# gisbi-kim/navtech-radar-slam

Hardware: AMD Instinct MI355X
Metric: sc_loop_queries_per_sec_vs_10k_scan_db (higher is better)
Workload: dtype f16 filter + f64 exact

## Files before the change

include/rsx_diag.h:

```cpp
#ifndef RSX_DIAG_H
#define RSX_DIAG_H

#include "rsx.h"

#ifdef __cplusplus
extern "C" {
#endif

int rsx_selftest_firewall(int kind);

int rsx_frontend_read_images(rsx_frontend *h, int32_t image, float *out_cart, float *out_blur);

int rsx_cen2018_gauss_weights(int32_t sigma_gauss, float *out, int32_t max);
int rsx_cen2018_debug_image(rsx_cen2018 *h, const uint8_t *img, int32_t row_stride, int32_t col_offset, const rsx_cen2018_params *params,
                            float *out_mean, float *out_sigma, float *out_p, float *out_y);

int rsx_sc_ringkey_tree_layout(const float *keys20, int64_t n, int32_t *out_vind, int32_t *out_n_nodes, int32_t *out_depth);

int rsx_sc_filter_bounds(rsx_sc *h, const float *q_descs, int32_t nq, float *out_lb);
double rsx_sc_filter_eps(void);

#define RSX_SC_WINDOW_P 320
#define RSX_SC_WINDOW_MARGIN 1.25e-3f
int rsx_sc_window_previews(rsx_sc *h, const float *q_descs, int32_t nq, int32_t k, int32_t *out_slots, float *out_pv,
                           int32_t *out_kstar, int32_t *out_shift_mask, int32_t *out_counts);

const char *rsx_sc_dominant_kernel_name(void);
const char *rsx_sc_profiled_kernel_name(rsx_sc *h);
int rsx_sc_profile_enable(rsx_sc *h, int on);
int rsx_sc_profile_read(rsx_sc *h, int64_t *launches, double *total_ms);
typedef struct {
  uint32_t struct_size;
  uint32_t reserved;
  int64_t candidates;
  int64_t exact_evals;
  int64_t queries_rescored;
  int64_t window_previews;
  int64_t valu_previews;
  int64_t exact_window_shifts;
} rsx_sc_rescoring_stats;
int rsx_sc_profile_read_rescoring(rsx_sc *h, rsx_sc_rescoring_stats *out);

#ifdef __cplusplus
}
#endif
#endif
```

navtech-radar-slam_amd/_rsx.py:

```python
import ctypes as C
import os

import numpy as np

_HERE = os.path.dirname(os.path.abspath(__file__))
LIB_PATH = os.environ.get("RSX_LIB_PATH") or os.path.join(_HERE, "librsx.so")

NUM_RING, NUM_SECTOR, DESC_SIZE, MAX_TOPK = 20, 60, 1200, 32
MODE_CANDIDATE, MODE_EXHAUSTIVE = 0, 1
FILTER_AUTO, FILTER_OFF, FILTER_FORCE, FILTER_Q1 = 0, 1, 2, 3
KIND_AUTO, KIND_DIRECT, KIND_SPECTRAL, KIND_SPECTRAL2 = 0, 1, 2, 3
SUM_EIGEN_SSE2, SUM_SEQ, SUM_EIGEN_AVX_FMA, SUM_EIGEN34_AVX_FMA = 0, 1, 2, 3
default_filter_kind = KIND_AUTO

HIT_DTYPE = np.dtype([("dist", "<f8"), ("index", "<i4"), ("shift", "<i4")])


class RsxError(RuntimeError):
    def __init__(self, status, msg):
        super().__init__(f"rsx status {status}: {msg}")
        self.status = status


class ScParams(C.Structure):
    _fields_ = [
        ("lidar_height", C.c_double),
        ("max_radius", C.c_double),
        ("num_exclude_recent", C.c_int32),
        ("num_candidates", C.c_int32),
        ("search_ratio", C.c_double),
        ("dist_thres", C.c_double),
        ("tree_making_period", C.c_int32),
        ("device", C.c_int32),
        ("shard_rank", C.c_int32),
        ("shard_world", C.c_int32),
        ("capacity_hint", C.c_int64),
        ("filter_mode", C.c_int32),
        ("filter_kind", C.c_int32),
        ("sum_order", C.c_int32),
    ]


class RescoringStats(C.Structure):
    _fields_ = [("struct_size", C.c_uint32), ("reserved", C.c_uint32), ("candidates", C.c_int64), ("exact_evals", C.c_int64),
                ("queries_rescored", C.c_int64), ("window_previews", C.c_int64), ("valu_previews", C.c_int64),
                ("exact_window_shifts", C.c_int64)]


ORORA_PMC = 4
ORORA_PMC_EXACT = 8
ORORA_PMC_PROVEN, ORORA_PMC_PASSTHROUGH, ORORA_PMC_NO_WORKSPACE, ORORA_PMC_MAXIMUM, ORORA_PMC_BUDGET = 1, 2, 4, 8, 16
PMC_INFO_DTYPE = np.dtype([("size", "<i4"), ("max_core", "<i4"), ("seeds", "<i4"), ("flags", "<i4")])


class ScDetection(C.Structure):
    _fields_ = [("loop_id", C.c_int32), ("yaw_diff_rad", C.c_float), ("min_dist", C.c_double), ("nn_idx", C.c_int32),
                ("query_idx", C.c_int32), ("searched", C.c_int32), ("reserved", C.c_int32), ("dist_thres", C.c_double)]


class OroraParams(C.Structure):
    _fields_ = [("tim_noise_bound", C.c_double), ("noise_bound_radial", C.c_double),
                ("noise_bound_tangential", C.c_double), ("gnc_factor", C.c_double),
                ("cost_threshold", C.c_double), ("max_iterations", C.c_int32), ("flags", C.c_int32)]


class IcpParams(C.Structure):
    _fields_ = [("max_corr_dist", C.c_double), ("transformation_epsilon", C.c_double),
                ("euclidean_fitness_epsilon", C.c_double), ("max_iterations", C.c_int32), ("flags", C.c_int32)]


class IcpResult(C.Structure):
    _fields_ = [("transform", C.c_float * 16), ("fitness", C.c_double), ("iterations", C.c_int32),
                ("converged", C.c_int32), ("state", C.c_int32), ("reserved", C.c_int32)]


class LoopVerifyParams(C.Structure):
    _fields_ = [("history_keyframe_search_num", C.c_int32), ("leaf", C.c_float), ("fitness_threshold", C.c_double), ("icp", IcpParams)]


class LoopVerifyResult(C.Structure):
    _fields_ = [("accepted", C.c_int32), ("converged", C.c_int32), ("iterations", C.c_int32), ("state", C.c_int32),
                ("fitness", C.c_double), ("transform", C.c_float * 16),
                ("x", C.c_float), ("y", C.c_float), ("z", C.c_float), ("roll", C.c_float), ("pitch", C.c_float), ("yaw", C.c_float),
                ("relative", C.c_double * 16), ("n_source", C.c_int64), ("n_target", C.c_int64)]


class FrontendParams(C.Structure):
    _fields_ = [("cart_pixel_width", C.c_int32), ("cart_resolution", C.c_float), ("ratio", C.c_float), ("flags", C.c_int32)]


class Cen2019Params(C.Structure):
    _fields_ = [("max_points", C.c_int32), ("min_range", C.c_int32)]


class Cen2018Params(C.Structure):
    _fields_ = [("zq", C.c_float), ("sigma_gauss", C.c_int32), ("min_range", C.c_int32), ("reserved", C.c_int32)]


class OroraResult(C.Structure):
# ... 261 lines not shown
```

navtech-radar-slam_amd/csrc/sc_api.cpp:

```cpp
#include <cmath>
#include <cstdio>
#include <cstdlib>
#include <cstring>
#include <mutex>
#include <new>
#include <string>
#include <vector>

#include "rsx_common.h"
#include "sc_kernels.h"
#include "sc_plan.h"
#include "sc_kdtree.h"
#include "loopverify.h"
#include "voxelgrid.h"

namespace rsx {
std::string &last_error() {
  static thread_local std::string e;
  return e;
}
}

using namespace rsx;
using namespace rsx::sc;
// ... 1489 lines not shown
    int count = 0;
    for (int p = 0; p < nparts; p++)
      for (int i = 0; i < k; i++) {
        const rsx_sc_hit &r = parts[((size_t)p * nq + q) * k + i];
        if (!(r.dist < 10000000)) continue;
        int pos = count < k ? count : k;
        while (pos > 0 && ((r.dist < o[pos - 1].dist) || (r.dist == o[pos - 1].dist && r.index < o[pos - 1].index))) pos--;
        if (pos >= k) continue;
        int last = count < k ? count : k - 1;
        for (int j = last; j > pos; j--) o[j] = o[j - 1];
        o[pos] = r;
        if (count < k) count++;
      }
    for (int i = count; i < k; i++) {
      o[i].dist = 10000000;
      o[i].index = 0;
      o[i].shift = 0;
    }
  }
  return RSX_OK;
} RSX_CATCH_ALL

int rsx_sc_merge_topk_device(rsx_sc *h, const rsx_sc_hit *d_parts, int32_t nparts, int32_t nq, int32_t k,
                             rsx_sc_hit *d_out, void *stream) try {
  if (!h || !d_parts || !d_out || nparts < 1 || nq < 1 || k < 1 || k > RSX_SC_MAX_TOPK) return fail(RSX_ERR_BAD_ARG, "bad arg");
  std::lock_guard<std::mutex> lk(h->mu);
  RSX_TRY(set_device(h));
  hipStream_t s;
  RSX_TRY(use_stream(h, stream, &s));
  return launch_merge(d_parts, nparts, nq, k, d_out, s);
} RSX_CATCH_ALL

int rsx_sc_profile_enable(rsx_sc *h, int on) try {
  if (!h) return fail(RSX_ERR_BAD_ARG, "null handle");
  std::lock_guard<std::mutex> lk(h->mu);
  RSX_TRY(own_stream(h));
  if (on && !h->prof.ev) {
    h->prof.ev.reset(new (std::nothrow) Event[2 * PairProfiler::kMax]);
    if (!h->prof.ev) return fail(RSX_ERR_OOM, "host alloc");
    for (int i = 0; i < 2 * PairProfiler::kMax; i++) RSX_HIP(h->prof.ev[i].create(true));
  }
  if (on) {
    RSX_TRY(h->stats.reserve(kStatBytes, h->stream, false));
    RSX_HIP(hipMemsetAsync(h->stats.p, 0, kStatBytes, h->stream));
    RSX_HIP(hipStreamSynchronize(h->stream));
  }
  h->prof.on = on != 0;
  h->prof.used = 0;
  return RSX_OK;
} RSX_CATCH_ALL

int rsx_sc_profile_read_rescoring(rsx_sc *h, rsx_sc_rescoring_stats *out) try {
  if (!h || !out || out->struct_size < offsetof(rsx_sc_rescoring_stats, candidates)) return fail(RSX_ERR_BAD_ARG, "null arg / struct_size not set");
  int64_t out6[6];
  int64_t *const out5 = out6;
  int64_t *candidates = out5, *exact_evals = out5 + 1, *queries_rescored = out5 + 2;
  struct Publish {
    rsx_sc_rescoring_stats *o;
    const int64_t *v;
    ~Publish() {
      int64_t *dst = &o->candidates;
      const size_t n = (o->struct_size - offsetof(rsx_sc_rescoring_stats, candidates)) / sizeof(int64_t);
      for (size_t i = 0; i < n && i < 6; i++) dst[i] = v[i];
    }
  } publish{out, out6};
  std::lock_guard<std::mutex> lk(h->mu);
  RSX_TRY(set_device(h));
  for (int i = 0; i < 6; i++) out6[i] = 0;
  if (!h->stats.p) return RSX_OK;
  RSX_HIP(hipDeviceSynchronize());
  unsigned long long v[RESCORE_STAT_WORDS] = {0};
  {
    std::vector<unsigned long long> all((size_t)RESCORE_STAT_COPIES * RESCORE_STAT_WORDS);
    RSX_HIP(hipMemcpy(all.data(), h->stats.p, kStatBytes, hipMemcpyDeviceToHost));
    RSX_HIP(hipMemset(h->stats.p, 0, kStatBytes));
    for (int c = 0; c < RESCORE_STAT_COPIES; c++)
      for (int i = 0; i < RESCORE_STAT_WORDS; i++) v[i] += all[(size_t)c * RESCORE_STAT_WORDS + i];
  }
  if (rsx::exp_env("RSX_RESCORE_PROF") && v[1])
    fprintf(stderr, "[sc_rescore prof] per query (cycles of wave 0): load %.0f  phaseA %.0f  mergeA %.0f  phaseB %.0f  mergeX %.0f  gather %.0f  total %.0f\n",
            (double)v[4] / v[1], (double)v[5] / v[1], (double)v[6] / v[1], (double)v[7] / v[1], (double)v[8] / v[1], (double)v[9] / v[1],
            (double)v[10] / v[1]);
  if (rsx::exp_env("RSX_RESCORE_PROF") && v[1] && v[13])
    fprintf(stderr, "[sc_rescore prof] wave kernel: header %.0f  records %.0f (then tau_ub = the 'phaseA' figure)\n", (double)v[13] / v[1], (double)v[14] / v[1]);
  *candidates = (int64_t)v[0];
  *exact_evals = v[2] ? (int64_t)v[2] : (int64_t)v[0];
  *queries_rescored = (int64_t)v[1];
  out5[3] = (int64_t)v[3];
  out5[4] = (int64_t)v[11];
  out6[5] = v[12] ? (int64_t)v[12] : 7 * *exact_evals;
  return RSX_OK;
} RSX_CATCH_ALL

int rsx_sc_profile_read(rsx_sc *h, int64_t *launches, double *total_ms) try {
  if (!h || !launches || !total_ms) return fail(RSX_ERR_BAD_ARG, "null arg");
  std::lock_guard<std::mutex> lk(h->mu);
  RSX_TRY(set_device(h));
  *launches = 0;
  *total_ms = 0.0;
  for (int i = 0; i < h->prof.used; i++) {
    RSX_HIP(hipEventSynchronize(h->prof.ev[2 * i + 1]));
    float ms = 0.f;
    RSX_HIP(hipEventElapsedTime(&ms, h->prof.ev[2 * i], h->prof.ev[2 * i + 1]));
    *total_ms += ms;
    (*launches)++;
  }
  h->prof.used = 0;
  return RSX_OK;
} RSX_CATCH_ALL

int rsx_sc_hit_to_loop(rsx_sc *h, const rsx_sc_hit *hit, int32_t *loop_id, float *yaw) try {
  if (!h || !hit) return fail(RSX_ERR_BAD_ARG, "null arg");
  std::lock_guard<std::mutex> lk(h->mu);
  if (loop_id) *loop_id = (hit->dist < h->p.dist_thres) ? hit->index : -1;
  if (yaw) *yaw = yaw_from_shift(hit->shift);
  return RSX_OK;
} RSX_CATCH_ALL

}
```

navtech-radar-slam_amd/csrc/sc_filter.hip:

```cpp
#include <hip/hip_runtime.h>

#include <cmath>
#include <cstdint>
#include <cstdlib>
#include <type_traits>
#include <utility>

#include "rsx_common.h"
#include "sc_kernels.h"
#include "sc_entry_dev.h"

namespace rsx {
namespace sc {

namespace {

typedef _Float16 half8 __attribute__((ext_vector_type(8)));
typedef float floatx16 __attribute__((ext_vector_type(16)));
typedef unsigned frag4 __attribute__((ext_vector_type(4)));
typedef unsigned long long u64;

#define AS1 __attribute__((address_space(1)))
#define AS3 __attribute__((address_space(3)))

// ... 267 lines not shown
      const uint4 *src = a.hnT + ((tile_ok ? tile : 0) * F_STEPS) * 64 + lane;
#pragma unroll
      for (int s = 0; s < F_STEPS; s++) {
        const uint4 v = src[s * 64];
        B[s] = *reinterpret_cast<const half8 *>(&v);
      }
#pragma unroll
      for (int s = F_B_VGPR; s < F_STEPS; s++) asm volatile("" : "+a"(B[s]));
    }
    const u64 m2 = n_ok ? a.cmask[n] : 0ull;
    const unsigned m2lo = (unsigned)m2, m2hi = (unsigned)(m2 >> 32) & 0x0fffffffu;

    asm volatile("s_waitcnt vmcnt(0)" ::: "memory");
    __syncthreads();

    floatx16 acc0, acc1, p0;
    frag4 first[F_DEPTH];
    int prev_q = -1;
    u64 prev_mask = 0;
    auto fin = [&](const Epi &ep) {
      float best = epi_end(ep);
      if ((prev_mask | m2) & kNonFinite) best = -INFINITY;
      if (n_ok && hh == 0) a.lb[(int64_t)prev_q * a.ld_lb + n] = lb_pack(best);
    };
    for (int p = 0; p < nphase; p++) {
      const int qp = q0 + p * F_QPP;
      if (p + 1 < nphase) {
        const int qn = qp + F_QPP;
        const int nqs = (q1 - qn < F_QPP) ? (q1 - qn) : F_QPP;
        stage_queries(a.qimg + (int64_t)qn * FILTER_QIMG_BYTES, smem + ((p + 1) & 1) * F_PHASE_BYTES,
                      nqs * FILTER_QIMG_BYTES, wave, lane);
      }
      const int nq_here = (q1 - qp < F_QPP) ? (q1 - qp) : F_QPP;
      if (tile_ok) {
        const unsigned phase_lds = lds_base + (unsigned)((p & 1) * F_PHASE_BYTES + aoff);
        first_prologue(first, phase_lds);
        for (int qq = 0; qq < nq_here; qq++) {
          const unsigned ap_lds = phase_lds + (unsigned)(qq * FILTER_QIMG_BYTES);
          const unsigned next_lds = (qq + 1 < nq_here) ? ap_lds + FILTER_QIMG_BYTES : ap_lds;
          const u64 cur_mask = *reinterpret_cast<const u64 *>(smem + (p & 1) * F_PHASE_BYTES + qq * FILTER_QIMG_BYTES + QIMG_MASK_OFF);
          if (prev_q < 0) filter_stage<true, false>(ap_lds, next_lds, first, B, acc0, acc1, p0, prev_mask, m2lo, m2hi, hh, fin);
          else filter_stage<true, true>(ap_lds, next_lds, first, B, acc0, acc1, p0, prev_mask, m2lo, m2hi, hh, fin);
          prev_q = qp + qq;
          prev_mask = cur_mask;
        }
      }
      asm volatile("s_waitcnt vmcnt(0)" ::: "memory");
      __syncthreads();
    }
    if (prev_q >= 0) filter_stage<false, true>(0u, 0u, first, B, acc0, acc1, p0, prev_mask, m2lo, m2hi, hh, fin);
  }
}

constexpr int H_BINS = 2048;
constexpr int SEL_U = 5;

__device__ __forceinline__ int lb_bin(float d) {
  if (!(d > 0.0f)) return 0;
  const float x = d * (float)H_BINS;
  return x >= (float)(H_BINS - 1) ? H_BINS - 1 : (int)x;
}

struct Elig {
  int64_t idx_base, idx_stride, n_eligible;
  const int64_t *q_elig;
};
__device__ __forceinline__ int64_t n_elig_items(const Elig &el, int q, int64_t n_items) {
  int64_t lim = el.n_eligible;
  if (el.q_elig) {
    const int64_t v = el.q_elig[q];
    lim = v < lim ? v : lim;
  }
  if (lim <= el.idx_base) return 0;
  const int64_t c = (lim - el.idx_base + el.idx_stride - 1) / el.idx_stride;
  return c < n_items ? c : n_items;
}

__device__ __forceinline__ float bin_edge(int b) {
  return b < 0 ? -INFINITY : (b >= H_BINS - 1 ? INFINITY : (float)(b + 1) / (float)H_BINS);
}

__global__ __launch_bounds__(256) void sc_select_kernel(const lb_t *__restrict__ lb, int64_t ld, int64_t n_items_all,
                                                        Elig el, int32_t first_target,
                                                        RescoreEntry *__restrict__ slist,
                                                        int32_t *__restrict__ sl_cnt, float *__restrict__ thr) {
  __shared__ int hist[H_BINS];
  __shared__ int wsum[4];
  __shared__ int s_bcap;
  __shared__ int s_total;
  const int q = blockIdx.x;
  const int lane = threadIdx.x & 63, wave = threadIdx.x >> 6;
  const lb_t *row = lb + (int64_t)q * ld;
  const int64_t n_items = n_elig_items(el, q, n_items_all);
  for (int i = threadIdx.x; i < H_BINS; i += 256) hist[i] = 0;
  if (threadIdx.x == 0) s_total = 0;
  __syncthreads();
  typedef _Float16 half8 __attribute__((ext_vector_type(8)));
  const uint4 *row8 = reinterpret_cast<const uint4 *>(row);
  const int64_t n8 = n_items >> 3;
  const bool one_piece = n8 <= 256 * SEL_U;
  uint4 keep[SEL_U];
  auto load_piece = [&](int64_t c0, uint4 (&x)[SEL_U]) {
#pragma unroll
    for (int u = 0; u < SEL_U; u++) {
      const int64_t j = c0 + u * 256 + threadIdx.x;
      x[u] = j < n8 ? row8[j] : uint4{0x7c007c00u, 0x7c007c00u, 0x7c007c00u, 0x7c007c00u};
    }
  };
  auto walk_piece = [&](int64_t c0, const uint4 (&x)[SEL_U], auto &&f) {
#pragma unroll
    for (int u = 0; u < SEL_U; u++) {
      const int64_t i = (c0 + u * 256 + threadIdx.x) << 3;
      const half8 h = __builtin_bit_cast(half8, x[u]);
#pragma unroll
      for (int e = 0; e < 8; e++) f((float)h[e], i + e);
    }
  };
  auto for_row = [&](bool first, auto &&f) {
    if (one_piece) {
      if (first) load_piece(0, keep);
      walk_piece(0, keep, f);
    } else {
      for (int64_t c0 = 0; c0 < n8; c0 += 256 * SEL_U) {
        uint4 x[SEL_U];
        load_piece(c0, x);
        walk_piece(c0, x, f);
      }
    }
    const int64_t i = (n8 << 3) + threadIdx.x;
    if (i < n_items) f((float)row[i], i);
  };
  for_row(true, [&](float d, int64_t) {
    if (d != INFINITY) atomicAdd(&hist[lb_bin(d)], 1);
  });
  __syncthreads();
  int v[8];
  int run = 0;
#pragma unroll
  for (int i = 0; i < 8; i++) {
    run += hist[threadIdx.x * 8 + i];
    v[i] = run;
  }
  int incl = run;
#pragma unroll
  for (int off = 1; off < 64; off <<= 1) {
    const int o = __shfl_up(incl, off);
    if (lane >= off) incl += o;
  }
  if (lane == 63) wsum[wave] = incl;
  __syncthreads();
  int base = incl - run;
  for (int w = 0; w < wave; w++) base += wsum[w];
  __syncthreads();
#pragma unroll
  for (int i = 0; i < 8; i++) hist[threadIdx.x * 8 + i] = base + v[i];
  __syncthreads();
  auto first_reaching = [&](int target) {
    int lo = 0, hi = H_BINS;
    while (lo < hi) {
      const int mid = (lo + hi) >> 1;
      if (hist[mid] >= target) hi = mid;
      else lo = mid + 1;
    }
    return lo;
  };
  if (threadIdx.x == 0) s_bcap = first_reaching(RESCORE_SHORTLIST_CAP + 1) - 1;
  __syncthreads();
  const int b_cap = s_bcap;
  if (threadIdx.x < RESCORE_NUM_THR) {
    int b = b_cap;
    if (threadIdx.x < RESCORE_NUM_THR - 1) {
      b = first_reaching(first_target << threadIdx.x);
      if (b > H_BINS - 1) b = H_BINS - 1;
      if (b > b_cap) b = b_cap;
    }
    thr[(int64_t)q * RESCORE_THR_STRIDE + threadIdx.x] = bin_edge(b);
    reinterpret_cast<int32_t *>(thr)[(int64_t)q * RESCORE_THR_STRIDE + RESCORE_NUM_THR + threadIdx.x] = b >= 0 ? hist[b] : 0;
  }
  RescoreEntry *out = slist + (int64_t)q * RESCORE_SHORTLIST_CAP;
  __shared__ int fill[H_BINS];
  for (int i = threadIdx.x; i < H_BINS; i += 256) fill[i] = i ? hist[i - 1] : 0;
  __syncthreads();
  if (b_cap >= 0) {
    for_row(false, [&](float d, int64_t i) {
      if (d == INFINITY) return;
      const int b = lb_bin(d);
      if (b > b_cap) return;
      RescoreEntry e;
      e.lb = d;
      e.slot = (int32_t)i;
      out[atomicAdd(&fill[b], 1)] = e;
    });
  }
  if (threadIdx.x == 0) s_total = b_cap >= 0 ? hist[b_cap] : 0;
  __syncthreads();
  if (threadIdx.x == 0) sl_cnt[q] = s_total;
}

__global__ __launch_bounds__(1024) void sc_filter_plan_kernel(Elig el, int32_t nq, int64_t n_items, int32_t qgroup,
                                                              int32_t *__restrict__ tb_qmin, int64_t *__restrict__ tb_cum) {
  __shared__ long long sh[1024];
  const int64_t ntb = (((n_items + 31) >> 5) + 3) >> 2;
  const int t = threadIdx.x;
  long long running = 0;
  for (int64_t base = 0; base < ntb; base += 1024) {
    const int64_t tb = base + t;
    long long items = 0;
    if (tb < ntb) {
      const int64_t g0 = el.idx_base + tb * 128 * el.idx_stride;
      int lo = 0, hi = nq;
      while (lo < hi) {
        const int mid = (lo + hi) >> 1;
        int64_t lim = el.n_eligible;
        if (el.q_elig) {
          const int64_t v = el.q_elig[mid];
          lim = v < lim ? v : lim;
        }
        if (lim > g0) hi = mid;
        else lo = mid + 1;
      }
      tb_qmin[tb] = lo / qgroup;
      items = (nq + qgroup - 1) / qgroup - lo / qgroup;
    }
    sh[t] = items;
    __syncthreads();
    for (int d = 1; d < 1024; d <<= 1) {
      const long long v = t >= d ? sh[t - d] : 0;
      __syncthreads();
      sh[t] += v;
      __syncthreads();
    }
    if (tb < ntb) tb_cum[tb] = running + sh[t] - items;
    running += sh[1023];
    __syncthreads();
  }
  if (t == 0) tb_cum[ntb] = running;
}

}

// ... 101 lines not shown
```

navtech-radar-slam_amd/csrc/sc_kernels.h:

```cpp
#pragma once
#include <hip/hip_runtime.h>

#include <cstdint>

#include "rsx_common.h"

namespace rsx {
namespace sc {

constexpr int NR = RSX_SC_NUM_RING;
constexpr int NS = RSX_SC_NUM_SECTOR;
constexpr int DS = RSX_SC_DESC_SIZE;

struct DbView {
  const float *desc;
  const double *vkey;
  const double *norm;
  const float *rkey;
  const void *hnT;
  const uint64_t *cmask;
  const void *spT;
  const float *sp_aux;
  const void *hnR;
  const void *vk16;
  const float *vk_n;
  int64_t n_local;
  int64_t idx_base;
  int64_t idx_stride;
  int32_t sum_order;
};

using lb_t = _Float16;
typedef _Float16 lb2_t __attribute__((ext_vector_type(2)));
#ifdef __HIPCC__
__device__ __forceinline__ lb_t lb_pack(float v) {
  return __builtin_bit_cast(lb2_t, __builtin_amdgcn_cvt_pkrtz(v, 0.0f))[0];
}
#endif

struct QueryView {
  const float *desc;
  const double *vkey;
  const double *norm;
  int32_t nq;
};

int launch_keys(const float *desc, int64_t n, double *vkey, double *norm, float *rkey, hipStream_t s, int sum_order);

int launch_build(const void *d_pts, int64_t n_pts, int64_t stride_bytes, double lidar_height,
                 double max_radius, float *out_desc, double *out_vkey, double *out_norm,
                 float *out_rkey, hipStream_t s, int sum_order);

int pair_num_slots(int64_t n_items, int32_t nq);
size_t pair_partial_bytes(int64_t n_items, int32_t nq, int32_t k);

int launch_pairs(const DbView &db, const QueryView &q, const int32_t *gather, int64_t first,
                 int64_t n_items, int64_t n_eligible, const int64_t *q_elig, double *out_dist,
                 int32_t *out_shift, rsx_sc_hit *d_partial, rsx_sc_hit *d_topk, int32_t k,
                 hipStream_t s);

int launch_insert(const void *d_pts, const int64_t *d_offs, int64_t n_pts, int64_t n_clouds, int64_t stride_bytes,
                  double lidar_height, double max_radius, int64_t first_slot, float *desc, double *vkey, double *norm,
                  float *rkey, void *hnT, void *hnR, uint64_t *cmask, void *spT, float *aux, void *vk16, float *vk_n,
                  hipStream_t s, int sum_order);

int launch_merge(const rsx_sc_hit *d_parts, int32_t nparts, int32_t nq, int32_t k, rsx_sc_hit *d_out,
                 hipStream_t s);

int launch_gather_bounds(const lb_t *d_blocks, int64_t block_ld, int64_t block_stride, int64_t q0, int32_t nq, lb_t *d_lb,
                         int64_t ld, hipStream_t s);

int launch_knn(const float *rkeys, int64_t n_search, const float *qkey, int32_t k, float *d_dist_ws,
               int32_t *out_idx, float *out_dist, int32_t *out_found, hipStream_t s);

constexpr int RESCORE_SHORTLIST_CAP = 2048;
constexpr int RESCORE_NUM_THR = 6;
constexpr int RESCORE_THR_STRIDE = 2 * RESCORE_NUM_THR;
constexpr int RESCORE_STAT_WORDS = 16, RESCORE_STAT_COPIES = 64;
struct WindowPreview;
struct RescoreEntry {
  float lb;
  int32_t slot;
};
int launch_select(const DbView &db, const lb_t *lb, int64_t ld_lb, int64_t n_items, int32_t nq, int64_t n_eligible,
                  const int64_t *q_elig, int32_t first_target, RescoreEntry *slist, int32_t *sl_cnt, float *thr,
                  hipStream_t s);
constexpr int RESCORE_ALL_ROUNDS = RESCORE_NUM_THR + 1;
int launch_rescore(const DbView &db, const QueryView &q, const lb_t *lb, int64_t ld_lb, int64_t n_items,
                   int64_t n_eligible, const int64_t *q_elig, const RescoreEntry *slist, const int32_t *sl_cnt,
                   const float *thr, double eps, int32_t round_begin, int32_t round_end, const rsx_sc_hit *tau_src,
                   const rsx_sc_hit *seed, rsx_sc_hit *d_out, int32_t k, hipStream_t s, unsigned long long *d_stats,
                   const WindowPreview *win);

constexpr int FILTER_QIMG_BYTES = 9984;
constexpr int FILTER_QIMG_ODD = 4960;
constexpr int FILTER_QIMG_MASK_OFF = 4928;
constexpr float FILTER_ACC_SCALE = 1073741824.0f;
constexpr int FILTER_DB_BYTES_PER_ENTRY = 2 * DS;
double filter_eps();
size_t filter_qimg_bytes(int32_t nq);
int launch_db_images(const float *desc, const double *norm, int64_t first, int64_t count, void *hnT, void *hnR,
                     uint64_t *cmask, hipStream_t s);
int launch_query_images(const float *desc, const double *norm, int32_t nq, void *qimg, hipStream_t s);
struct FilterPlanInput {
  int64_t n_eligible;
  const int64_t *q_elig;
};
size_t filter_plan_bytes(int64_t n_items);
int launch_filter_plan(const DbView &db, const FilterPlanInput &plan, int32_t nq, int64_t n_items, int32_t qgroup,
                       void *plan_ws, const int32_t **tb_qmin, const int64_t **tb_cum, hipStream_t s);
int launch_filter(const DbView &db, const void *qimg, int32_t nq, int64_t n_items, lb_t *lb, int64_t ld_lb,
                  const FilterPlanInput *plan, void *plan_ws, hipStream_t s);
const char *pair_kernel_name();
const char *filter_kernel_name();

constexpr int SPEC_QIMG_BYTES = 4736;
constexpr int SPEC_DB_BYTES_PER_ENTRY = 2432;
size_t spec_qimg_bytes(int32_t nq);
int launch_spec_db_images(const float *desc, const double *norm, int64_t first, int64_t count, void *spT, float *aux,
                          hipStream_t s);
int launch_spec_query_images(const float *desc, const double *norm, int32_t nq, void *qimg, hipStream_t s);
int launch_spec_filter(const DbView &db, const void *qimg, int32_t nq, int64_t n_items, lb_t *lb, int64_t ld_lb,
                       const int32_t *tb_qmin, const int64_t *tb_cum, hipStream_t s, bool two_waves);
const char *spec_filter_kernel_name();
const char *spec2_filter_kernel_name();

constexpr int WINDOW_P = RSX_SC_WINDOW_P;
constexpr int WINDOW_HEAD = 128;
constexpr float WINDOW_MARGIN = RSX_SC_WINDOW_MARGIN;
constexpr int WINDOW_QK_BYTES = 4624;
static_assert(WINDOW_P % 64 == 0 && WINDOW_HEAD == 128 && WINDOW_P > WINDOW_HEAD, "layout");
// ... 31 lines not shown
```

navtech-radar-slam_amd/csrc/sc_kernels.hip:

```cpp
#include <hip/hip_runtime.h>

#include <cmath>
#include <cstdint>
#include <cstdio>
#include <cstdlib>

#include "rsx_common.h"
#include "sc_kernels.h"
#include "sc_entry_dev.h"
#include "sc_exact_dev.h"

namespace rsx {
namespace sc {

namespace {

using dev::wave_keys;


template <int SO>
__global__ __launch_bounds__(256) void sc_keys_kernel(const float *__restrict__ desc, int64_t n,
                                                      double *__restrict__ vkey, double *__restrict__ norm,
                                                      float *__restrict__ rkey) {
  const int lane = threadIdx.x & 63;
// ... 821 lines not shown
}

int launch_pairs(const DbView &db, const QueryView &q, const int32_t *gather, int64_t first,
                 int64_t n_items, int64_t n_eligible, const int64_t *q_elig, double *out_dist,
                 int32_t *out_shift, rsx_sc_hit *d_partial, rsx_sc_hit *d_topk, int32_t k,
                 hipStream_t s) {
  if (q.nq <= 0) return RSX_OK;
  if (k < 0 || k > RSX_SC_MAX_TOPK) return fail(RSX_ERR_BAD_ARG, "k=%d out of range [0,%d]", k, RSX_SC_MAX_TOPK);
  if (n_items <= 0) {
    if (d_topk && k > 0) {
      hipLaunchKernelGGL(sc_merge_kernel, dim3(q.nq), dim3(64), 0, s, (const rsx_sc_hit *)nullptr, 0,
                         (int64_t)0, (int64_t)k, k, k, d_topk);
      RSX_HIP(hipGetLastError());
    }
    return RSX_OK;
  }
  PairArgs a;
  a.db = db;
  a.q = q;
  a.gather = gather;
  a.first = first;
  a.n_items = n_items;
  a.n_eligible = n_eligible < 0 ? INT64_MAX : n_eligible;
  a.q_elig = q_elig;
  a.out_dist = out_dist;
  a.out_shift = out_shift;
  const int gx = choose_gx(n_items, q.nq);
  a.partial = (d_topk && k > 0) ? d_partial : nullptr;
  a.k = k;
  a.nslots = gx * 4;
  PairProfiler *pp = (g_prof && g_prof->on && g_prof->ev && g_prof->used < PairProfiler::kMax) ? g_prof : nullptr;
  if (pp) RSX_HIP(hipEventRecord(pp->ev[2 * pp->used], s));
  if (a.partial && !out_dist) {
    static_assert(PAIR2_LDS <= 48 * 1024, "within the default dynamic LDS limit: no per-device opt-in needed");
    RSX_SO_DISPATCH(db.sum_order, hipLaunchKernelGGL((sc_pair2_kernel<4, SO>), dim3(gx, q.nq), dim3(256), PAIR2_LDS, s, a));
    RSX_HIP(hipGetLastError());
  } else {
    int st = RSX_OK;
    RSX_SO_DISPATCH(db.sum_order, st = (launch_pairs_t<kPairB, kPairW, SO>(a, gx, s)));
    RSX_TRY(st);
  }
  if (pp) {
    RSX_HIP(hipEventRecord(pp->ev[2 * pp->used + 1], s));
    pp->used++;
  }
  if (a.partial) {
    hipLaunchKernelGGL(sc_merge_kernel, dim3(q.nq), dim3(64), 0, s, (const rsx_sc_hit *)d_partial, 1,
                       (int64_t)0, (int64_t)a.nslots * k, a.nslots * k, k, d_topk);
    RSX_HIP(hipGetLastError());
  }
  return RSX_OK;
}

__device__ __forceinline__ float bound_bin_lo(float lb) {
  if (!(lb > 0.0f)) return -INFINITY;
  const float x = lb * 2048.0f;
  return x >= 2047.0f ? 2047.0f / 2048.0f : floorf(x) / 2048.0f;
}

constexpr int RW_CH = (WINDOW_P + 63) / 64;


#ifndef RW_OCC
#define RW_OCC 3
#endif
template <int SO>
__global__ __launch_bounds__(64, RW_OCC) void sc_rescore_wave_kernel(RescoreArgs a) {
  extern __shared__ __attribute__((aligned(16))) char smem[];
  if (a.stats) a.stats += (blockIdx.x % RESCORE_STAT_COPIES) * RESCORE_STAT_WORDS;
  const int lane = threadIdx.x;
  const int qi = blockIdx.x;
  char *wsm = smem + WaveLds::OFF_ENT;

  int64_t n_elig = a.n_eligible;
  if (a.q_elig) {
    const int64_t e = a.q_elig[qi];
    n_elig = e < n_elig ? e : n_elig;
  }
  int64_t n_rows = 0;
  if (n_elig > a.db.idx_base) {
    n_rows = (n_elig - a.db.idx_base + a.db.idx_stride - 1) / a.db.idx_stride;
    n_rows = n_rows < a.n_items ? n_rows : a.n_items;
  }

  double ld = INFINITY;
  int li = 0x7fffffff, ls = 0;
  double tau_init = INFINITY;
  if (a.tau_src) {
    const double d = a.tau_src[(int64_t)qi * a.k + (a.k - 1)].dist;
    if (d < kBig) tau_init = d;
  }
  if (a.seed && lane < a.k) {
    const rsx_sc_hit h = a.seed[(int64_t)qi * a.k + lane];
    if (h.dist < kBig) {
      ld = h.dist; li = h.index; ls = h.shift;
    }
  }
  auto kth_of = [&](double list) {
    const double t = __shfl(list, a.k - 1);
    return t < tau_init ? t : tau_init;
  };
  double tau = kth_of(ld);
  bool query_loaded = false;
  unsigned n_exact = 0, n_looked = 0, n_aligned = 0, n_shifts = 0;
  unsigned nl_lane = 0, n_windowed = 0;

#ifdef RSX_EXPERIMENTS
  const bool timing = a.stats != nullptr;
#else
  constexpr bool timing = false;
#endif
  long long tacc[9] = {0, 0, 0, 0, 0, 0, 0, 0, 0};
  long long t_mark = timing ? clock64() : 0;
  const long long t_begin = t_mark;
  auto lap = [&](int slot_) {
    if (!timing) return;
    const long long t = clock64();
    tacc[slot_] += t - t_mark;
    t_mark = t;
  };
  auto eval = [&](int64_t slot, int ksm, const EntryRegs &er) {
    if (timing) {
      lap(2);
      asm volatile("s_waitcnt vmcnt(0)" ::: "memory");
      lap(5);
    }
    int ks = ksm;
    unsigned tmask = 0x7fu;
    if (ksm >= 0) {
      ks = ksm & 63;
      const unsigned m7 = ((unsigned)ksm >> 8) & 0x7fu;
      if (m7) tmask = m7;
    }
    if (!query_loaded) {
      const float4 *src = reinterpret_cast<const float4 *>(a.q.desc + (int64_t)qi * DS);
      float4 *dst = reinterpret_cast<float4 *>(smem + WaveLds::OFF_QF32);
      float4 x[5];
#pragma unroll
      for (int i = 0; i < 5; i++) x[i] = (lane + 64 * i < DS / 4) ? src[lane + 64 * i] : float4{0.f, 0.f, 0.f, 0.f};
      const double kn = lane < NS ? a.q.norm[(int64_t)qi * NS + lane] : 0.0;
      const double kv = lane < NS ? a.q.vkey[(int64_t)qi * NS + lane] : 0.0;
#pragma unroll
      for (int i = 0; i < 5; i++)
        if (lane + 64 * i < DS / 4) dst[lane + 64 * i] = x[i];
      if (lane < NS) {
        reinterpret_cast<double *>(smem + WaveLds::OFF_QN1)[lane] = kn;
        reinterpret_cast<double *>(smem + WaveLds::OFF_QV1)[lane] = kv;
      }
      query_loaded = true;
      wave_lds_fence();
      lap(0);
    }
    if (ks < 0) {
      ks = align_exact<SO>(reinterpret_cast<const double *>(smem + WaveLds::OFF_QV1), wsm, lane, er.v);
      n_aligned++;
      lap(4);
    }
    double bd;
// ... 109 lines not shown
          cbuf[rank] = Packed{lo[j], i0 + lane + 64 * j};
          lo[j] = INFINITY;
        }
        nsurv += __popcll(bal);
      }
      if (nsurv == 0) break;
      nsurv = nsurv < 64 ? nsurv : 64;
      wave_lds_fence();
      float mylo = INFINITY;
      int32_t myslot = 0;
      int myks = -1;
      if (lane < nsurv) {
        const Packed c = cbuf[lane];
        mylo = c.lo;
        myslot = sl[c.pos].slot;
        const int k_ = wp[c.pos].ks;
        myks = k_ >= 0 ? k_ : -1;
      }
      wave_lds_fence();
      {
        Touch tch;
        for (int i = 0; i < nsurv; i++) touch_entry(a.db, __shfl(myslot, i), lane, tch);
        touch_wait(tch);
      }
      auto pick = [&](int32_t &slot, int &ks) -> float {
        const float wm = wave_min_f32(mylo);
        if (wm == INFINITY) return wm;
        const int src = __ffsll((long long)__ballot(mylo == wm)) - 1;
        slot = __shfl(myslot, src);
        ks = __shfl(myks, src);
        if (lane == src) mylo = INFINITY;
        return wm;
      };
      EntryRegs cur, nxt;
      int32_t cur_slot = 0, nxt_slot = 0;
      int cur_ks = -1, nxt_ks = -1;
      float cur_lo = pick(cur_slot, cur_ks);
      if (cur_lo < INFINITY) load_entry(a.db, cur_slot, lane, cur);
      while (cur_lo < INFINITY) {
        const double t_eff = tau < tau_ub ? tau : tau_ub;
        if ((double)cur_lo > t_eff) break;
        const float nxt_lo = pick(nxt_slot, nxt_ks);
        if (nxt_lo < INFINITY && !((double)nxt_lo > t_eff)) load_entry(a.db, nxt_slot, lane, nxt);
        eval(cur_slot, cur_ks, cur);
        cur_lo = nxt_lo;
        cur_slot = nxt_slot;
        cur_ks = nxt_ks;
        cur = nxt;
      }
    }
    pos_next = pw > i0 ? pw : i0;
  }

  for (int base = pos_next; base < i1 && !done; base += 64) {
    const int n_here = (i1 - base < 64) ? (i1 - base) : 64;
    RescoreEntry mine;
    mine.lb = INFINITY;
    mine.slot = 0;
    if (lane < n_here) mine = sl[base + lane];
    for (int i = 0; i < n_here; i++) {
      const float lb = __shfl(mine.lb, i);
      const int32_t slot = __shfl(mine.slot, i);
      if ((double)bound_bin_lo(lb) - a.eps > tau) {
        done = true;
        break;
      }
      if ((double)lb - a.eps > tau) continue;
      const int64_t gidx = a.db.idx_base + (int64_t)slot * a.db.idx_stride;
      if (!(gidx < n_elig)) continue;
      EntryRegs er;
      load_entry(a.db, slot, lane, er);
      n_looked++;
      eval(slot, -1, er);
    }
  }

  if (!done && a.round_end > RESCORE_NUM_THR && t_cap < INFINITY && !((double)t_cap - a.eps > tau)) {
    const lb_t *row = a.lb + (int64_t)qi * a.ld_lb;
    const bool take_all = (t_cap == -INFINITY);
    for (int64_t pos = 0; pos < n_rows; pos += 64) {
      const int64_t i = pos + lane;
      const float d = (i < n_rows) ? (float)row[i] : INFINITY;
      const bool beyond = take_all ? true : (d >= t_cap);
      unsigned long long bal = __ballot((i < n_rows) && beyond && (d != INFINITY));
      while (bal) {
        const int l = __ffsll((long long)bal) - 1;
        bal &= bal - 1;
        const float dl = __shfl(d, l);
        if ((double)dl - a.eps > tau) continue;
        EntryRegs er;
        load_entry(a.db, pos + l, lane, er);
        n_looked++;
        eval(pos + l, -1, er);
      }
    }
  }

  if (lane < a.k) {
    rsx_sc_hit h;
    if (ld == INFINITY) {
      h.dist = kBig; h.index = 0; h.shift = 0;
    } else {
      h.dist = ld; h.index = li; h.shift = ls;
    }
    a.out[(int64_t)qi * a.k + lane] = h;
  }
  if (a.stats) {
    unsigned lk = nl_lane, wd = n_windowed;
#pragma unroll
    for (int off = 32; off >= 1; off >>= 1) {
      lk += __shfl_xor(lk, off);
      wd += __shfl_xor(wd, off);
    }
    if (lane == 0) {
      atomicAdd(a.stats, (unsigned long long)(lk + n_looked));
      atomicAdd(a.stats + 3, (unsigned long long)wd);
      atomicAdd(a.stats + 2, (unsigned long long)n_exact);
      atomicAdd(a.stats + 11, (unsigned long long)n_aligned);
      atomicAdd(a.stats + 12, (unsigned long long)n_shifts);
      if (timing) {
        for (int i = 0; i < 6; i++) atomicAdd(a.stats + 4 + i, (unsigned long long)tacc[i]);
        atomicAdd(a.stats + 13, (unsigned long long)tacc[7]);
        atomicAdd(a.stats + 14, (unsigned long long)tacc[8]);
        atomicAdd(a.stats + 10, (unsigned long long)(clock64() - t_begin));
      }
      if (n_exact) atomicAdd(a.stats + 1, 1ull);
    }
  }
}

int launch_rescore(const DbView &db, const QueryView &q, const lb_t *lb, int64_t ld_lb, int64_t n_items,
                   int64_t n_eligible, const int64_t *q_elig, const RescoreEntry *slist, const int32_t *sl_cnt,
                   const float *thr, double eps, int32_t round_begin, int32_t round_end, const rsx_sc_hit *tau_src,
                   const rsx_sc_hit *seed, rsx_sc_hit *d_out, int32_t k, hipStream_t s, unsigned long long *d_stats,
                   const WindowPreview *win) {
  if (q.nq <= 0) return RSX_OK;
  if (k < 1 || k > RSX_SC_MAX_TOPK) return fail(RSX_ERR_BAD_ARG, "k=%d out of range [1,%d]", k, RSX_SC_MAX_TOPK);
  RescoreArgs a;
  a.db = db;
  a.q = q;
  a.lb = lb;
  a.ld_lb = ld_lb;
  a.n_items = n_items;
  a.n_eligible = n_eligible < 0 ? INT64_MAX : n_eligible;
  a.q_elig = q_elig;
  a.slist = slist;
  a.sl_cnt = sl_cnt;
  a.thr = thr;
  a.out = d_out;
  a.tau_src = tau_src;
  a.seed = seed;
  a.eps = eps;
  a.k = k;
  a.round_begin = round_begin;
  a.round_end = round_end;
  a.stats = d_stats;
  a.win = win;
  RSX_SO_DISPATCH(db.sum_order, hipLaunchKernelGGL(sc_rescore_wave_kernel<SO>, dim3(q.nq), dim3(64), WaveLds::SIZE, s, a));
  RSX_HIP(hipGetLastError());
  return RSX_OK;
}

int launch_knn(const float *rkeys, int64_t n_search, const float *qkey, int32_t k, float *d_dist_ws,
               int32_t *out_idx, float *out_dist, int32_t *out_found, hipStream_t s) {
  hipLaunchKernelGGL(sc_knn_kernel, dim3(1), dim3(1024), 0, s, rkeys, n_search, qkey, k, d_dist_ws, out_idx,
                     out_dist, out_found);
  RSX_HIP(hipGetLastError());
  return RSX_OK;
}

}
}
// ... 1 lines not shown
```

navtech-radar-slam_amd/scancontext.py:

```python
import ctypes as C
import os

import numpy as np

from . import _rsx
from ._rsx import HIT_DTYPE, MODE_CANDIDATE, MODE_EXHAUSTIVE, check, lib

WINDOW_P = 320
WINDOW_MARGIN = 1.25e-3


class SCManager:
    LIDAR_HEIGHT = 2.0
    PC_NUM_RING = 20
    PC_NUM_SECTOR = 60
    PC_MAX_RADIUS = 80.0
    NUM_EXCLUDE_RECENT = 30
    NUM_CANDIDATES_FROM_TREE = 3
    SEARCH_RATIO = 0.1
    TREE_MAKING_PERIOD_ = 30

    def __init__(self, device=0, shard_rank=0, shard_world=1, capacity_hint=1024, sc_dist_thres=0.2,
                 lidar_height=None, num_exclude_recent=None, num_candidates=None, tree_making_period=None,
                 filter_mode=_rsx.FILTER_AUTO, filter_kind=_rsx.KIND_AUTO, sum_order=_rsx.SUM_EIGEN_SSE2):
# ... 213 lines not shown

    def pair_distances(self, q_desc, first=0, count=None):
        q = np.ascontiguousarray(q_desc, dtype=np.float32).reshape(-1)
        if count is None:
            count = self.local_size - first
        dist = np.empty(count, dtype=np.float64)
        shift = np.empty(count, dtype=np.int32)
        check(self._L.rsx_sc_pair_distances(self._h, q.ctypes.data, first, count, dist.ctypes.data, shift.ctypes.data))
        return dist, shift

    def filter_bounds(self, q_descs):
        q = np.ascontiguousarray(q_descs, dtype=np.float32).reshape(-1, 1200)
        out = np.empty((q.shape[0], self.local_size), dtype=np.float32)
        check(self._L.rsx_sc_filter_bounds(self._h, q.ctypes.data, q.shape[0], out.ctypes.data))
        return out

    def window_previews(self, q_descs, k=10):
        q = np.ascontiguousarray(q_descs, dtype=np.float32).reshape(-1, 1200)
        nq = q.shape[0]
        slots = np.empty((nq, WINDOW_P), dtype=np.int32)
        pv = np.empty((nq, WINDOW_P), dtype=np.float32)
        ks = np.empty((nq, WINDOW_P), dtype=np.int32)
        sm = np.empty((nq, WINDOW_P), dtype=np.int32)
        cnt = np.empty(nq, dtype=np.int32)
        check(self._L.rsx_sc_window_previews(self._h, q.ctypes.data, nq, k, slots.ctypes.data, pv.ctypes.data, ks.ctypes.data,
                                             sm.ctypes.data, cnt.ctypes.data))
        return slots, pv, ks, sm, cnt

    @staticmethod
    def filter_eps():
        return lib().rsx_sc_filter_eps()

    def profiled_kernel_name(self):
        return self._L.rsx_sc_profiled_kernel_name(self._h).decode()

    def merge_device(self, parts_ptr, nparts, nq, k, out_ptr, stream=0):
        check(self._L.rsx_sc_merge_topk_device(self._h, parts_ptr, nparts, nq, k, out_ptr, stream))

    def profile_enable(self, on=True):
        check(self._L.rsx_sc_profile_enable(self._h, 1 if on else 0))

    def profile_read(self):
        n, ms = C.c_int64(), C.c_double()
        check(self._L.rsx_sc_profile_read(self._h, C.byref(n), C.byref(ms)))
        return n.value, ms.value

    def profile_read_rescoring(self):
        from ._rsx import RescoringStats
        st = RescoringStats()
        st.struct_size = C.sizeof(RescoringStats)
        check(self._L.rsx_sc_profile_read_rescoring(self._h, C.byref(st)))
        return (st.candidates, st.exact_evals, st.queries_rescored, st.window_previews, st.valu_previews, st.exact_window_shifts)

    def hit_to_loop(self, hit):
        h = np.zeros(1, dtype=HIT_DTYPE)
        h[0] = hit
        lid, yaw = C.c_int32(), C.c_float()
        check(self._L.rsx_sc_hit_to_loop(self._h, h.ctypes.data, C.byref(lid), C.byref(yaw)))
        return lid.value, yaw.value


class ShardedSet:

    def __init__(self, devices, sc_dist_thres=0.2, capacity_hint=1024, query_groups=1, exchange="peer"):
        L = lib()
        p = _rsx.ScParams()
        check(L.rsx_sc_default_params(C.byref(p)))
        p.dist_thres = sc_dist_thres
        p.capacity_hint = capacity_hint
        dev = (C.c_int32 * len(devices))(*devices)
        self._h = C.c_void_p()
        self._L = L
        check(L.rsx_scs_create_layout(C.byref(p), dev, len(devices), query_groups, {"peer": 0, "rccl": 1}[exchange], C.byref(self._h)))

    def close(self):
        if getattr(self, "_h", None) and self._h.value:
            self._L.rsx_scs_destroy(self._h)
            self._h = C.c_void_p()

    def __del__(self):
        try:
            self.close()
        except Exception:
            pass

    @property
    def num_shards(self):
        return self._L.rsx_scs_num_shards(self._h)

    @property
    def num_query_groups(self):
        return self._L.rsx_scs_num_query_groups(self._h)

    def __len__(self):
        n = C.c_int64()
        check(self._L.rsx_scs_size(self._h, C.byref(n)))
        return n.value

    def makeAndSaveScancontextAndKeys(self, scan_down):
        pts = np.ascontiguousarray(scan_down, dtype=np.float32)
        idx = C.c_int32()
        check(self._L.rsx_scs_add_points(self._h, pts.ctypes.data, pts.shape[0], pts.shape[1] * 4, C.byref(idx)))
        return idx.value

    def add_descriptors_f32(self, descs):
        d = np.ascontiguousarray(descs, dtype=np.float32).reshape(-1, 1200)
# ... 26 lines not shown
```

Measured before the change: 3.188 million.

## Cap shortlist at a head and walk the tail bins by rescanning bounds

The select kernel now writes only the first bins up to a head of 512 entries into the per-query shortlist and records the head bin and end. The rescore kernel processes that head as before. If the threshold is not yet tight, it walks the remaining bins by rescanning the f16 lower-bound row bin by bin, taking the minimum next bin each pass. The goal is to shrink the shortlist writes and the scatter work in the select kernel, since most queries stop early. In exchange, queries that need the tail pay one full-row rescan per bin. The change also adds tail stats counters and bumps the threshold stride and stat word count.

```diff
diff --git a/include/rsx_diag.h b/include/rsx_diag.h
--- a/include/rsx_diag.h
+++ b/include/rsx_diag.h
@@ -38,6 +38,8 @@
   int64_t window_previews;
   int64_t valu_previews;
   int64_t exact_window_shifts;
+  int64_t tail_evals;
+  int64_t tail_queries;
 } rsx_sc_rescoring_stats;
 int rsx_sc_profile_read_rescoring(rsx_sc *h, rsx_sc_rescoring_stats *out);
 
diff --git a/navtech-radar-slam_amd/_rsx.py b/navtech-radar-slam_amd/_rsx.py
--- a/navtech-radar-slam_amd/_rsx.py
+++ b/navtech-radar-slam_amd/_rsx.py
@@ -45,6 +45,10 @@
     _fields_ = [("struct_size", C.c_uint32), ("reserved", C.c_uint32), ("candidates", C.c_int64), ("exact_evals", C.c_int64),
                 ("queries_rescored", C.c_int64), ("window_previews", C.c_int64), ("valu_previews", C.c_int64),
                 ("exact_window_shifts", C.c_int64)]
+
+
+class RescoringStatsTail(RescoringStats):
+    _fields_ = [("tail_evals", C.c_int64), ("tail_queries", C.c_int64)]
 
 
 ORORA_PMC = 4
diff --git a/navtech-radar-slam_amd/csrc/sc_api.cpp b/navtech-radar-slam_amd/csrc/sc_api.cpp
--- a/navtech-radar-slam_amd/csrc/sc_api.cpp
+++ b/navtech-radar-slam_amd/csrc/sc_api.cpp
@@ -1565,7 +1565,7 @@
 
 int rsx_sc_profile_read_rescoring(rsx_sc *h, rsx_sc_rescoring_stats *out) try {
   if (!h || !out || out->struct_size < offsetof(rsx_sc_rescoring_stats, candidates)) return fail(RSX_ERR_BAD_ARG, "null arg / struct_size not set");
-  int64_t out6[6];
+  int64_t out6[8];
   int64_t *const out5 = out6;
   int64_t *candidates = out5, *exact_evals = out5 + 1, *queries_rescored = out5 + 2;
   struct Publish {
@@ -1574,12 +1574,12 @@
     ~Publish() {
       int64_t *dst = &o->candidates;
       const size_t n = (o->struct_size - offsetof(rsx_sc_rescoring_stats, candidates)) / sizeof(int64_t);
-      for (size_t i = 0; i < n && i < 6; i++) dst[i] = v[i];
+      for (size_t i = 0; i < n && i < 8; i++) dst[i] = v[i];
     }
   } publish{out, out6};
   std::lock_guard<std::mutex> lk(h->mu);
   RSX_TRY(set_device(h));
-  for (int i = 0; i < 6; i++) out6[i] = 0;
+  for (int i = 0; i < 8; i++) out6[i] = 0;
   if (!h->stats.p) return RSX_OK;
   RSX_HIP(hipDeviceSynchronize());
   unsigned long long v[RESCORE_STAT_WORDS] = {0};
@@ -1602,6 +1602,8 @@
   out5[3] = (int64_t)v[3];
   out5[4] = (int64_t)v[11];
   out6[5] = v[12] ? (int64_t)v[12] : 7 * *exact_evals;
+  out6[6] = (int64_t)v[15];
+  out6[7] = (int64_t)v[16];
   return RSX_OK;
 } RSX_CATCH_ALL
 
diff --git a/navtech-radar-slam_amd/csrc/sc_filter.hip b/navtech-radar-slam_amd/csrc/sc_filter.hip
--- a/navtech-radar-slam_amd/csrc/sc_filter.hip
+++ b/navtech-radar-slam_amd/csrc/sc_filter.hip
@@ -343,14 +343,8 @@
   }
 }
 
-constexpr int H_BINS = 2048;
+constexpr int H_BINS = RESCORE_BINS;
 constexpr int SEL_U = 5;
-
-__device__ __forceinline__ int lb_bin(float d) {
-  if (!(d > 0.0f)) return 0;
-  const float x = d * (float)H_BINS;
-  return x >= (float)(H_BINS - 1) ? H_BINS - 1 : (int)x;
-}
 
 struct Elig {
   int64_t idx_base, idx_stride, n_eligible;
@@ -367,9 +361,6 @@
   return c < n_items ? c : n_items;
 }
 
-__device__ __forceinline__ float bin_edge(int b) {
-  return b < 0 ? -INFINITY : (b >= H_BINS - 1 ? INFINITY : (float)(b + 1) / (float)H_BINS);
-}
 
 __global__ __launch_bounds__(256) void sc_select_kernel(const lb_t *__restrict__ lb, int64_t ld, int64_t n_items_all,
                                                         Elig el, int32_t first_target,
@@ -465,18 +456,25 @@
       if (b > H_BINS - 1) b = H_BINS - 1;
       if (b > b_cap) b = b_cap;
     }
-    thr[(int64_t)q * RESCORE_THR_STRIDE + threadIdx.x] = bin_edge(b);
+    thr[(int64_t)q * RESCORE_THR_STRIDE + threadIdx.x] = lb_bin_edge(b);
     reinterpret_cast<int32_t *>(thr)[(int64_t)q * RESCORE_THR_STRIDE + RESCORE_NUM_THR + threadIdx.x] = b >= 0 ? hist[b] : 0;
+  }
+  int b_head = first_reaching(RESCORE_HEAD);
+  if (b_head > b_cap) b_head = b_cap;
+  if (threadIdx.x == 0) {
+    int32_t *hd = reinterpret_cast<int32_t *>(thr) + (int64_t)q * RESCORE_THR_STRIDE;
+    hd[RESCORE_THR_HEAD_BIN] = b_head;
+    hd[RESCORE_THR_HEAD_END] = b_head >= 0 ? hist[b_head] : 0;
   }
   RescoreEntry *out = slist + (int64_t)q * RESCORE_SHORTLIST_CAP;
   __shared__ int fill[H_BINS];
   for (int i = threadIdx.x; i < H_BINS; i += 256) fill[i] = i ? hist[i - 1] : 0;
   __syncthreads();
-  if (b_cap >= 0) {
+  if (b_head >= 0) {
     for_row(false, [&](float d, int64_t i) {
       if (d == INFINITY) return;
       const int b = lb_bin(d);
-      if (b > b_cap) return;
+      if (b > b_head) return;
       RescoreEntry e;
       e.lb = d;
       e.slot = (int32_t)i;
diff --git a/navtech-radar-slam_amd/csrc/sc_kernels.h b/navtech-radar-slam_amd/csrc/sc_kernels.h
--- a/navtech-radar-slam_amd/csrc/sc_kernels.h
+++ b/navtech-radar-slam_amd/csrc/sc_kernels.h
@@ -32,9 +32,24 @@
 
 using lb_t = _Float16;
 typedef _Float16 lb2_t __attribute__((ext_vector_type(2)));
+constexpr int RESCORE_BINS = 2048;
 #ifdef __HIPCC__
 __device__ __forceinline__ lb_t lb_pack(float v) {
   return __builtin_bit_cast(lb2_t, __builtin_amdgcn_cvt_pkrtz(v, 0.0f))[0];
+}
+__device__ __forceinline__ int lb_bin(float d) {
+  if (!(d > 0.0f)) return 0;
+  const float x = d * (float)RESCORE_BINS;
+  return x >= (float)(RESCORE_BINS - 1) ? RESCORE_BINS - 1 : (int)x;
+}
+__device__ __forceinline__ float lb_bin_edge(int b) {
+  return b < 0 ? -INFINITY : (b >= RESCORE_BINS - 1 ? INFINITY : (float)(b + 1) / (float)RESCORE_BINS);
+}
+__device__ __forceinline__ int lb_edge_bin(float edge) {
+  return edge == -INFINITY ? -1 : (edge == INFINITY ? RESCORE_BINS - 1 : (int)(edge * (float)RESCORE_BINS) - 1);
+}
+__device__ __forceinline__ float lb_bin_lo(int b) {
+  return b <= 0 ? -INFINITY : (float)b / (float)RESCORE_BINS;
 }
 #endif
 
@@ -74,9 +89,14 @@
                int32_t *out_idx, float *out_dist, int32_t *out_found, hipStream_t s);
 
 constexpr int RESCORE_SHORTLIST_CAP = 2048;
+constexpr int RESCORE_HEAD = 512;
+static_assert(RESCORE_HEAD >= RSX_SC_WINDOW_P && RESCORE_HEAD <= RESCORE_SHORTLIST_CAP,
+              "the head must cover every list position sc_window_kernel may read (WINDOW_P)");
 constexpr int RESCORE_NUM_THR = 6;
-constexpr int RESCORE_THR_STRIDE = 2 * RESCORE_NUM_THR;
-constexpr int RESCORE_STAT_WORDS = 16, RESCORE_STAT_COPIES = 64;
+constexpr int RESCORE_THR_HEAD_BIN = 2 * RESCORE_NUM_THR, RESCORE_THR_HEAD_END = 2 * RESCORE_NUM_THR + 1;
+constexpr int RESCORE_THR_STRIDE = 16;
+static_assert(RESCORE_THR_HEAD_END < RESCORE_THR_STRIDE, "layout");
+constexpr int RESCORE_STAT_WORDS = 24, RESCORE_STAT_COPIES = 64;
 struct WindowPreview;
 struct RescoreEntry {
   float lb;
diff --git a/navtech-radar-slam_amd/csrc/sc_kernels.hip b/navtech-radar-slam_amd/csrc/sc_kernels.hip
--- a/navtech-radar-slam_amd/csrc/sc_kernels.hip
+++ b/navtech-radar-slam_amd/csrc/sc_kernels.hip
@@ -897,11 +897,6 @@
   return RSX_OK;
 }
 
-__device__ __forceinline__ float bound_bin_lo(float lb) {
-  if (!(lb > 0.0f)) return -INFINITY;
-  const float x = lb * 2048.0f;
-  return x >= 2047.0f ? 2047.0f / 2048.0f : floorf(x) / 2048.0f;
-}
 
 constexpr int RW_CH = (WINDOW_P + 63) / 64;
 
@@ -947,8 +942,9 @@
   };
   double tau = kth_of(ld);
   bool query_loaded = false;
-  unsigned n_exact = 0, n_looked = 0, n_aligned = 0, n_shifts = 0;
+  unsigned n_exact = 0, n_looked = 0, n_aligned = 0, n_shifts = 0, n_tail = 0;
   unsigned nl_lane = 0, n_windowed = 0;
+  bool walked_tail = false;
 
 #ifdef RSX_EXPERIMENTS
   const bool timing = a.stats != nullptr;
@@ -1164,8 +1160,10 @@
     pos_next = pw > i0 ? pw : i0;
   }
 
-  for (int base = pos_next; base < i1 && !done; base += 64) {
-    const int n_here = (i1 - base < 64) ? (i1 - base) : 64;
+  const int head_bin = rcnt[RESCORE_THR_HEAD_BIN - RESCORE_NUM_THR], head_end = rcnt[RESCORE_THR_HEAD_END - RESCORE_NUM_THR];
+  const int i1h = i1 < head_end ? i1 : head_end;
+  for (int base = pos_next; base < i1h && !done; base += 64) {
+    const int n_here = (i1h - base < 64) ? (i1h - base) : 64;
     RescoreEntry mine;
     mine.lb = INFINITY;
     mine.slot = 0;
@@ -1173,7 +1171,7 @@
     for (int i = 0; i < n_here; i++) {
       const float lb = __shfl(mine.lb, i);
       const int32_t slot = __shfl(mine.slot, i);
-      if ((double)bound_bin_lo(lb) - a.eps > tau) {
+      if ((double)lb_bin_lo(lb_bin(lb)) - a.eps > tau) {
         done = true;
         break;
       }
@@ -1184,6 +1182,62 @@
       load_entry(a.db, slot, lane, er);
       n_looked++;
       eval(slot, -1, er);
+    }
+  }
+
+  if (!done && i1 > head_end) {
+    const lb_t *row = a.lb + (int64_t)qi * a.ld_lb;
+    const int b_to = lb_edge_bin(thr[r_end - 1]);
+    int b = head_bin;
+    if (a.round_begin > 0) {
+      const int b0 = lb_edge_bin(thr[(a.round_begin < RESCORE_NUM_THR ? a.round_begin : RESCORE_NUM_THR) - 1]);
+      b = b0 > b ? b0 : b;
+    }
+    bool take = false;
+    walked_tail = b < b_to;
+    while (!done && walked_tail) {
+      int next = RESCORE_BINS;
+      constexpr int U = 4;
+      for (int64_t pos = 0; pos < n_rows && !done; pos += 64 * U) {
+        float d[U];
+#pragma unroll
+        for (int u = 0; u < U; u++) {
+          const int64_t i = pos + 64 * u + lane;
+          d[u] = (i < n_rows) ? (float)row[i] : INFINITY;
+        }
+#pragma unroll
+        for (int u = 0; u < U; u++) {
+          const int bin = (d[u] != INFINITY) ? lb_bin(d[u]) : RESCORE_BINS;
+          if (bin > b && bin < next) next = bin;
+          unsigned long long bal = __ballot(take && bin == b);
+          while (bal && !done) {
+            const int l = __ffsll((long long)bal) - 1;
+            bal &= bal - 1;
+            if ((double)lb_bin_lo(b) - a.eps > tau) {
+              done = true;
+              break;
+            }
+            const float dl = __shfl(d[u], l);
+            if ((double)dl - a.eps > tau) continue;
+            const int64_t slot = pos + 64 * u + l;
+            EntryRegs er;
+            load_entry(a.db, slot, lane, er);
+            n_looked++;
+            n_tail++;
+            eval(slot, -1, er);
+          }
+        }
+      }
+      if (done) break;
+#pragma unroll
+      for (int off = 32; off >= 1; off >>= 1) {
+        const int o = __shfl_xor(next, off);
+        next = o < next ? o : next;
+      }
+      if (next > b_to) break;
+      b = next;
+      take = true;
+      if ((double)lb_bin_lo(b) - a.eps > tau) done = true;
     }
   }
 
@@ -1230,6 +1284,8 @@
       atomicAdd(a.stats + 2, (unsigned long long)n_exact);
       atomicAdd(a.stats + 11, (unsigned long long)n_aligned);
       atomicAdd(a.stats + 12, (unsigned long long)n_shifts);
+      atomicAdd(a.stats + 15, (unsigned long long)n_tail);
+      if (walked_tail) atomicAdd(a.stats + 16, 1ull);
       if (timing) {
         for (int i = 0; i < 6; i++) atomicAdd(a.stats + 4 + i, (unsigned long long)tacc[i]);
         atomicAdd(a.stats + 13, (unsigned long long)tacc[7]);
diff --git a/navtech-radar-slam_amd/scancontext.py b/navtech-radar-slam_amd/scancontext.py
--- a/navtech-radar-slam_amd/scancontext.py
+++ b/navtech-radar-slam_amd/scancontext.py
@@ -289,6 +289,14 @@
         check(self._L.rsx_sc_profile_read_rescoring(self._h, C.byref(st)))
         return (st.candidates, st.exact_evals, st.queries_rescored, st.window_previews, st.valu_previews, st.exact_window_shifts)
 
+    def profile_read_rescoring_tail(self):
+        from ._rsx import RescoringStats, RescoringStatsTail
+        st = RescoringStatsTail()
+        st.struct_size = C.sizeof(RescoringStatsTail)
+        check(self._L.rsx_sc_profile_read_rescoring(self._h, C.cast(C.byref(st), C.POINTER(RescoringStats))))
+        return (st.candidates, st.exact_evals, st.queries_rescored, st.window_previews, st.valu_previews, st.exact_window_shifts,
+                st.tail_evals, st.tail_queries)
+
     def hit_to_loop(self, hit):
         h = np.zeros(1, dtype=HIT_DTYPE)
         h[0] = hit
```

Result: faster. 3.230 million, median of 6 (+1.3%).
